# xmed-lab/NEURONS

Measured on AMD Instinct MI355X. Metric: denoising frames/sec, 16f x 256^2 clip, 50 DDIM steps, higher is better.
Workload: dtype bf16; 1 GPU; BASELINE config 2: 1 clip(s) per call, (1,4,16,32,32) latent, 50 DDIM steps, CFG 8.5 (batch 2), SparseCtrl + temporal U-Net per step, random-init weights; clips_per_gpu=5, ddim_steps=50, hip_graph=True, output_finite=True, attention=bf16

## Files before the change

### neurons_amd/csrc/gemm.hip

```cpp
#include "launchers.h"
#include "device_prims.h"
#include <cstdio>
#include <cstdlib>
#include <utility>

namespace {

__device__ __forceinline__ void glds16_builtin(const void* src, void* lds_wave_base) {
  __builtin_amdgcn_global_load_lds((gptr_t)src, (lptr_t)lds_wave_base, 16, 0, 0);
}

NR_STAMP_BUF(nr_stamp_buf, 512, 48);
#define NR_STAMP_AT(slot) NR_STAMP_PUT(nr_stamp_buf, slot)
#define NR_STAMP_RT(slot) NR_STAMP_PUT_RT(nr_stamp_buf, slot)

template <int BM, int BN, int NS, int WGM, int WGN, bool LNF = false, bool ADMA = false, bool LIN = LNF, bool PH = false>
__global__ __launch_bounds__(64 * WGM * WGN, (LNF && WGM * WGN == 8) ? 4 : 1) void igemm_bf16_kernel(NrGemmParams p_arg, int splitk, float* partial, int m_fast) {
  NrGemmParams p = nr_pin_params(p_arg);
  if constexpr (LIN) { p.ksize = 1; p.stride = 1; p.ups = 0; p.a1 = nullptr; p.c1 = 0; p.tap_inner = 0; p.pad_tl0 = 0; }
  static_assert(!PH || (!LIN && !LNF), "the phase form is a conv");
  if constexpr (PH) { p.ksize = 3; p.stride = 1; p.ups = 2; p.a1 = nullptr; p.c1 = 0; p.tap_inner = 0; p.pad_tl0 = 0; p.geglu = 0; p.rowvec = nullptr; p.res = nullptr; }
  splitk = nr_pin(splitk); partial = nr_pin(partial); m_fast = nr_pin(m_fast);
  constexpr int BK = 64;
  constexpr int NW = WGM * WGN;
  constexpr int WM = BM / WGM, WN = BN / WGN;
  constexpr int MT = WM / 16, NT = WN / 16;
  constexpr int GA = BM / (8 * NW), GB = BN / (8 * NW);
  static_assert(BM % (8 * NW) == 0 && BN % (8 * NW) == 0, "tile rows must split evenly over the waves");
  constexpr int TILE = (BM + BN) * BK;
  extern __shared__ __attribute__((aligned(16))) bf16 smem[];

  const int tid = threadIdx.x;
  const int lane = tid & 63;
  const int wave = tid >> 6;
  NR_STAMP_AT(0);
  NR_STAMP_RT(44);
  const int wm = wave / WGN, wn = wave % WGN;
  const int ntn = (p.N + BN - 1) / BN;
  const int Mrows = PH ? p.M >> 2 : p.M;
  const int ntmp = (Mrows + BM - 1) / BM;
  const int ntm = PH ? 4 * ntmp : ntmp;
  int bid = nr_xcd_bid();
  const int slice = splitk > 1 ? nr_fdiv_small(bid, ntn * ntm) : 0;
  bid -= slice * ntn * ntm;
  int bm, bn;
  if (m_fast >= 2) {
    const int G = m_fast;
    const int band = nr_fdiv_small(bid, G * ntn);
    const int first = band * G;
    const int gsz = min(G, ntm - first);
    const int r = bid - band * G * ntn;
    bn = nr_fdiv_small(r, gsz);
    bm = first + r - bn * gsz;
  } else if (m_fast) { bn = nr_fdiv_small(bid, ntm); bm = bid - bn * ntm; } else { bm = nr_fdiv_small(bid, ntn); bn = bid - bm * ntn; }
  const int phase = PH ? nr_fdiv_small(bm, ntmp) : 0;
  if constexpr (PH) bm -= phase * ntmp;
  const int ph_py = phase >> 1, ph_px = phase & 1;
  const int m0 = bm * BM, n0 = bn * BN;
  auto ph_out_row = [&](int r) {
    const int hw = p.H * p.W;
    const int n = nr_fdiv_small(r, hw);
    const int q = r - n * hw;
    const int y = nr_fdiv_small(q, p.W), x = q - y * p.W;
    return (n * p.OH + 2 * y + ph_py) * p.OW + 2 * x + ph_px;
  };
  NR_STAMP_AT(40);
  const int lr = lane >> 3;
  const int lp = lane & 7;
  const int lchunk = (lp ^ lr) << 3;

  const int Cin = p.c0 + p.c1;

  int a_pix[GA], a_oy[GA], a_ox[GA];
  bool a_ok[GA];
#pragma unroll
  for (int j = 0; j < GA; ++j) {
    const int m = m0 + 8 * (wave * GA + j) + lr;
    a_ok[j] = m < Mrows;
    const int mm = a_ok[j] ? m : 0;
    if constexpr (PH) {
      const int hw = p.H * p.W;
      const int n = nr_fdiv_small(mm, hw);
      const int r = mm - n * hw;
      a_pix[j] = n; a_oy[j] = nr_fdiv_small(r, p.W); a_ox[j] = r - a_oy[j] * p.W;
    } else if (p.ksize == 1) {
      a_pix[j] = mm; a_oy[j] = 0; a_ox[j] = 0;
    } else {
      const int ohw = p.OH * p.OW;
      const int n = nr_fdiv_small(mm, ohw);
      const int r = mm - n * ohw;
      a_pix[j] = n; a_oy[j] = nr_fdiv_small(r, p.OW); a_ox[j] = r - a_oy[j] * p.OW;
    }
  }
  const bf16* zsrc = (const bf16*)nr_zero16;
  const bool tap_inner = !LNF && p.tap_inner != 0;
  long long a_cbyte[GA];
  unsigned a_tapmask[GA];
  if (tap_inner) {
#pragma unroll
    for (int j = 0; j < GA; ++j) {
      a_cbyte[j] = (((long long)a_pix[j] * p.H + a_oy[j]) * p.W + a_ox[j]) * p.lda0 * (long long)sizeof(bf16);
      unsigned msk = 0;
#pragma unroll
      for (int t = 0; t < 9; ++t) {
        const int iy = a_oy[j] + t / 3 - 1, ix = a_ox[j] + t % 3 - 1;
        if (a_ok[j] && iy >= 0 && iy < p.H && ix >= 0 && ix < p.W) msk |= 1u << t;
      }
      a_tapmask[j] = msk;
    }
  }

  NR_STAMP_AT(41);
  const int nk_total = p.K / BK;
  int kt_begin = 0, kt_end = nk_total;
  if (splitk > 1) { kt_begin = nr_fdiv_small(nk_total * slice, splitk); kt_end = nr_fdiv_small(nk_total * (slice + 1), splitk); }

  const bf16* ap[GA];
  int ainc[GA];
  const bf16* wp[GB];
  int winc[GB];
  int st_tap, st_c;
  {
    const int kbase = kt_begin * BK;
    if (tap_inner) { const int q9 = nr_fdiv_small(kt_begin, 9); st_tap = kt_begin - 9 * q9; st_c = q9 * BK; }
    else { st_tap = p.ksize == 3 ? nr_fdiv_small(kbase, Cin) : 0; st_c = kbase - st_tap * Cin; }
#pragma unroll
    for (int j = 0; j < GB; ++j) {
      const int n = n0 + 8 * (wave * GB + j) + lr;
      const bool ok = n < p.N;
      wp[j] = ok ? p.w + ((size_t)phase * p.N + n) * p.K + kbase + lchunk : zsrc;
      winc[j] = ok ? BK : 0;
    }
  }
  auto setup_rows_tap_inner = [&]() {
    const int ky = st_tap / 3, kx = st_tap - ky * 3;
    const long long delta = ((long long)(ky - 1) * p.W + (kx - 1)) * p.lda0 * (long long)sizeof(bf16);
    const char* base = reinterpret_cast<const char*>(p.a0 + st_c + lchunk) + delta;
#pragma unroll
    for (int j = 0; j < GA; ++j) {
      const bool ok = (a_tapmask[j] >> st_tap) & 1u;
      ap[j] = ok ? reinterpret_cast<const bf16*>(base + a_cbyte[j]) : zsrc;
    }
  };
  auto setup_rows = [&]() {
    if (tap_inner) { setup_rows_tap_inner(); return; }
    const bf16* src; int ld;
    if (st_c < p.c0) { src = p.a0 + st_c; ld = p.lda0; } else { src = p.a1 + (st_c - p.c0); ld = p.lda1; }
    src += lchunk;
    if constexpr (PH) {
      const int dy = (st_tap >> 1) + ph_py - 1, dx = (st_tap & 1) + ph_px - 1;
#pragma unroll
      for (int j = 0; j < GA; ++j) {
        const int iy = a_oy[j] + dy, ix = a_ox[j] + dx;
        const bool ok = a_ok[j] && iy >= 0 && iy < p.H && ix >= 0 && ix < p.W;
        const size_t pix = ((size_t)a_pix[j] * p.H + iy) * p.W + ix;
        ap[j] = ok ? src + pix * ld : zsrc;
        ainc[j] = ok ? BK : 0;
      }
    } else if (p.ksize == 1) {
#pragma unroll
      for (int j = 0; j < GA; ++j) {
        ap[j] = a_ok[j] ? src + (size_t)a_pix[j] * ld : zsrc;
        ainc[j] = a_ok[j] ? BK : 0;
      }
    } else {
      const int ky = st_tap / 3, kx = st_tap - ky * 3;
      const int VH = p.ups ? p.H * 2 : p.H, VW = p.ups ? p.W * 2 : p.W;
#pragma unroll
      for (int j = 0; j < GA; ++j) {
        int iy = a_oy[j] * p.stride + ky - (p.pad_tl0 ? 0 : 1);
        int ix = a_ox[j] * p.stride + kx - (p.pad_tl0 ? 0 : 1);
        const bool ok = a_ok[j] && iy >= 0 && iy < VH && ix >= 0 && ix < VW;
        if (p.ups) { iy >>= 1; ix >>= 1; }
        const size_t pix = ((size_t)a_pix[j] * p.H + iy) * p.W + ix;
        ap[j] = ok ? src + pix * ld : zsrc;
        ainc[j] = ok ? BK : 0;
      }
    }
  };
  NR_STAMP_AT(42);
  setup_rows();
  NR_STAMP_AT(43);

  auto stage = [&](int buf) {
    bf16* sA = smem + buf * TILE;
    bf16* sB = sA + BM * BK;
    if constexpr (ADMA) {
      const unsigned la = nr_lds_addr(sA + wave * GA * 8 * BK), lb = nr_lds_addr(sB + wave * GB * 8 * BK);
#pragma unroll
      for (int j = 0; j < GA; ++j) nr_glds16(ap[j], la + (unsigned)(j * 8 * BK * (int)sizeof(bf16)));
#pragma unroll
      for (int j = 0; j < GB; ++j) nr_glds16(wp[j], lb + (unsigned)(j * 8 * BK * (int)sizeof(bf16)));
    } else {
#pragma unroll
      for (int j = 0; j < GA; ++j) glds16_builtin(ap[j], sA + (wave * GA + j) * 8 * BK);
#pragma unroll
      for (int j = 0; j < GB; ++j) glds16_builtin(wp[j], sB + (wave * GB + j) * 8 * BK);
    }
#pragma unroll
    for (int j = 0; j < GB; ++j) wp[j] += winc[j];
    if (tap_inner) {
      st_tap += 1;
      if (st_tap == 9) { st_tap = 0; st_c += BK; }
      setup_rows_tap_inner();
      return;
    }
    st_c += BK;
    bool resetup = false;
    if (st_c == Cin) { st_c = 0; st_tap += 1; resetup = true; }
    else if (p.c1 > 0 && st_c == p.c0) resetup = true;
    if (resetup) {
      if (st_tap < (PH ? 4 : p.ksize * p.ksize)) setup_rows();
    } else {
#pragma unroll
      for (int j = 0; j < GA; ++j) ap[j] += ainc[j];
    }
  };

  f32x4 acc[NT][MT];
#pragma unroll
  for (int i = 0; i < NT; ++i)
#pragma unroll
    for (int j = 0; j < MT; ++j) acc[i][j] = f32x4{0.f, 0.f, 0.f, 0.f};

  const int fr = lane & 15, fg = lane >> 4;
  float ln_s1[MT], ln_s2[MT];
#pragma unroll
  for (int j = 0; j < MT; ++j) { ln_s1[j] = 0.f; ln_s2[j] = 0.f; }
  float* ln_stat = reinterpret_cast<float*>(smem + NS * TILE);

  constexpr int G = GA + GB;
#pragma unroll
  for (int s0 = 0; s0 < NS - 1; ++s0)
    if (kt_begin + s0 < kt_end) stage(s0);
  int cur = 0;
  NR_STAMP_AT(1);
  for (int kt = kt_begin; kt < kt_end; ++kt) {
    if (kt + (NS - 2) < kt_end) nr_wait_vmcnt<(NS - 2) * G>(); else nr_wait_vmcnt<0>();
    __builtin_amdgcn_s_barrier();
    NR_STAMP_AT(4 + (kt - kt_begin));
    const bf16* sA = smem + cur * TILE;
    const bf16* sB = sA + BM * BK;
    bf16x8 wf[2][NT], xf[2][MT];
#pragma unroll
    for (int i = 0; i < NT; ++i) {
      const int row = wn * WN + i * 16 + fr;
      wf[0][i] = *(const bf16x8*)(sB + row * BK + ((fg ^ (row & 7)) << 3));
    }
#pragma unroll
    for (int j = 0; j < MT; ++j) {
      const int row = wm * WM + j * 16 + fr;
      xf[0][j] = *(const bf16x8*)(sA + row * BK + ((fg ^ (row & 7)) << 3));
    }
    __builtin_amdgcn_sched_barrier(0);
    {
      const int nxt = kt + NS - 1;
      int nb = cur + NS - 1; if (nb >= NS) nb -= NS;
      if (nxt < kt_end) stage(nb);
    }
    __builtin_amdgcn_sched_barrier(0);
#pragma unroll
    for (int i = 0; i < NT; ++i) {
      const int row = wn * WN + i * 16 + fr;
      wf[1][i] = *(const bf16x8*)(sB + row * BK + (((4 + fg) ^ (row & 7)) << 3));
    }
#pragma unroll
    for (int j = 0; j < MT; ++j) {
      const int row = wm * WM + j * 16 + fr;
      xf[1][j] = *(const bf16x8*)(sA + row * BK + (((4 + fg) ^ (row & 7)) << 3));
    }
#pragma unroll
    for (int ks = 0; ks < 2; ++ks)
#pragma unroll
      for (int i = 0; i < NT; ++i)
#pragma unroll
        for (int j = 0; j < MT; ++j)
          acc[i][j] = __builtin_amdgcn_mfma_f32_16x16x32_bf16(wf[ks][i], xf[ks][j], acc[i][j], 0, 0, 0);
    if constexpr (LNF) {
      const bf16x2 one2 = {(bf16)1.0f, (bf16)1.0f};
#pragma unroll
      for (int ks = 0; ks < 2; ++ks) {
        if (((2 * kt + ks) & (WGN - 1)) != wn) continue;
#pragma unroll
        for (int j = 0; j < MT; ++j)
#pragma unroll
          for (int e = 0; e < 4; ++e) {
            const bf16x2 pr = {xf[ks][j][2 * e], xf[ks][j][2 * e + 1]};
            ln_s2[j] = __builtin_amdgcn_fdot2_f32_bf16(pr, pr, ln_s2[j], false);
            ln_s1[j] = __builtin_amdgcn_fdot2_f32_bf16(pr, one2, ln_s1[j], false);
          }
      }
    }
    cur = cur + 1 == NS ? 0 : cur + 1;
  }
  NR_STAMP_AT(2);
  float ln_mu[MT], ln_rs[MT];
  if constexpr (LNF) {
#pragma unroll
    for (int j = 0; j < MT; ++j) {
      float a = ln_s1[j], b = ln_s2[j];
      a += __shfl_xor(a, 16, 64); b += __shfl_xor(b, 16, 64);
      a += __shfl_xor(a, 32, 64); b += __shfl_xor(b, 32, 64);
      if (fg == 0) {
        const int row = wm * WM + j * 16 + fr;
        ln_stat[(0 * WGN + wn) * BM + row] = a;
        ln_stat[(1 * WGN + wn) * BM + row] = b;
      }
    }
    __syncthreads();
#pragma unroll
    for (int j = 0; j < MT; ++j) {
      const int row = wm * WM + j * 16 + fr;
      float a = 0.f, b = 0.f;
#pragma unroll
      for (int w = 0; w < WGN; ++w) { a += ln_stat[(0 * WGN + w) * BM + row]; b += ln_stat[(1 * WGN + w) * BM + row]; }
      const float inv = 1.0f / (float)p.K;
      const float mu = a * inv;
      ln_mu[j] = mu;
      ln_rs[j] = rsqrtf(fmaxf(b * inv - mu * mu, 0.f) + p.ln_eps);
    }
#pragma unroll
    for (int i = 0; i < NT; ++i) {
      const int n = n0 + wn * WN + i * 16 + 4 * fg;
      const f32x4 cn = n < p.N ? *(const f32x4*)(p.ln_c + n) : f32x4{0.f, 0.f, 0.f, 0.f};
#pragma unroll
      for (int j = 0; j < MT; ++j)
#pragma unroll
        for (int r = 0; r < 4; ++r) acc[i][j][r] = ln_rs[j] * (acc[i][j][r] - ln_mu[j] * cn[r]);
    }
  }

  if (partial) {
    float* slab = partial + (size_t)slice * p.M * p.N;
#pragma unroll
    for (int j = 0; j < MT; ++j) {
      const int m = m0 + wm * WM + j * 16 + fr;
      if (m >= Mrows) continue;
      const int ms = PH ? phase * Mrows + m : m;
#pragma unroll
      for (int i = 0; i < NT; ++i) {
        const int n = n0 + wn * WN + i * 16 + 4 * fg;
        if (n >= p.N) continue;
        nr_store16f(slab + (size_t)ms * p.N + n, acc[i][j]);
      }
    }
    return;
  }
  constexpr bool STAGED = (size_t)BM * BN * sizeof(float) <= (size_t)NS * TILE * sizeof(bf16);
  if constexpr (STAGED) {
    constexpr int NTH = 64 * NW;
    float* sC = reinterpret_cast<float*>(smem);
    __syncthreads();
    const int bno = p.geglu ? BN / 2 : BN;
#pragma unroll
    for (int j = 0; j < MT; ++j) {
      const int row = wm * WM + j * 16 + fr;
      if (!p.geglu) {
#pragma unroll
        for (int i = 0; i < NT; ++i) {
          const int c4 = ((wn * WN + i * 16) >> 2) + fg;
          *(f32x4*)(sC + row * BN + ((c4 ^ (row & 7)) << 2)) = acc[i][j];
        }
      } else {
        if constexpr (NT % 2 == 0) {
#pragma unroll
          for (int i = 0; i < NT; i += 2) {
            const int nv = n0 + wn * WN + i * 16 + 4 * fg;
            f32x4 v = acc[i][j], g = acc[i + 1][j];
            if (p.bias && nv < p.N) { v += *(const f32x4*)(p.bias + nv); g += *(const f32x4*)(p.bias + nv + 16); }
            f32x4 o;
#pragma unroll
            for (int e = 0; e < 4; ++e) o[e] = v[e] * gelu_erf_fast(g[e]);
            const int c4 = (((wn * WN + i * 16) >> 1) >> 2) + fg;
            *(f32x4*)(sC + row * BN + ((c4 ^ (row & 7)) << 2)) = o;
          }
        }
      }
    }
    __syncthreads();
    const int c8n = bno >> 3;
    const int nout = p.geglu ? p.N / 2 : p.N;
    const int nb0 = p.geglu ? n0 / 2 : n0;
    for (int idx = tid; idx < BM * c8n; idx += NTH) {
      const int row = idx / c8n, c8 = idx - row * c8n;
      const int m = m0 + row, n = nb0 + c8 * 8;
      if (m >= Mrows || n >= nout) continue;
      f32x4 va = *(const f32x4*)(sC + row * BN + (((2 * c8) ^ (row & 7)) << 2));
      f32x4 vb = *(const f32x4*)(sC + row * BN + (((2 * c8 + 1) ^ (row & 7)) << 2));
      if (!p.geglu) {
        if (p.bias) { va += *(const f32x4*)(p.bias + n); vb += *(const f32x4*)(p.bias + n + 4); }
        if (p.rowvec) {
          const float* rv = p.rowvec + nr_rowvec_row(p, m) + n;
          va += *(const f32x4*)rv; vb += *(const f32x4*)(rv + 4);
        }
        va *= p.out_scale; vb *= p.out_scale;
        if (p.act == 1) {
#pragma unroll
          for (int e = 0; e < 4; ++e) { va[e] = quick_gelu_f(va[e]); vb[e] = quick_gelu_f(vb[e]); }
        }
        if (p.res) {
          const bf16x8 r = *(const bf16x8*)(p.res + (size_t)m * p.ldr + n);
#pragma unroll
          for (int e = 0; e < 4; ++e) { va[e] += (float)r[e]; vb[e] += (float)r[4 + e]; }
        }
      }
      bf16x8 o;
#pragma unroll
      for (int e = 0; e < 4; ++e) { o[e] = (bf16)va[e]; o[4 + e] = (bf16)vb[e]; }
      nr_store16(p.out + (size_t)(PH ? ph_out_row(m) : m) * p.ldo + n, o);
    }
#ifdef NR_STAMP
    asm volatile("s_waitcnt vmcnt(0)" ::: "memory");
#endif
    NR_STAMP_AT(3);
    NR_STAMP_RT(45);
    return;
  }
#pragma unroll
  for (int j = 0; j < MT; ++j) {
    const int m = m0 + wm * WM + j * 16 + fr;
    if (m >= Mrows) continue;
    const size_t mo = PH ? ph_out_row(m) : m;
    const float* rv = p.rowvec ? p.rowvec + nr_rowvec_row(p, m) : nullptr;
    if (!p.geglu) {
#pragma unroll
      for (int i = 0; i < NT; ++i) {
        const int n = n0 + wn * WN + i * 16 + 4 * fg;
        if (n >= p.N) continue;
        f32x4 v = acc[i][j];
        if (p.bias) { const f32x4 b = *(const f32x4*)(p.bias + n); v += b; }
        if (rv) { const f32x4 t = *(const f32x4*)(rv + n); v += t; }
        v *= p.out_scale;
        if (p.act == 1) {
#pragma unroll
          for (int e = 0; e < 4; ++e) v[e] = quick_gelu_f(v[e]);
        }
        if (p.res) {
          const bf16x4 r = *(const bf16x4*)(p.res + (size_t)m * p.ldr + n);
#pragma unroll
          for (int e = 0; e < 4; ++e) v[e] += (float)r[e];
        }
        bf16x4 o;
#pragma unroll
        for (int e = 0; e < 4; ++e) o[e] = (bf16)v[e];
        nr_store8(p.out + mo * p.ldo + n, o);
      }
    } else {
      if constexpr (NT % 2 == 0) {
#pragma unroll
        for (int i = 0; i < NT; i += 2) {
          const int nv = n0 + wn * WN + i * 16 + 4 * fg;
          if (nv >= p.N) continue;
          const int ng = nv + 16;
          f32x4 v = acc[i][j], g = acc[i + 1][j];
          if (p.bias) {
            v += *(const f32x4*)(p.bias + nv);
            g += *(const f32x4*)(p.bias + ng);
          }
          const int oc = ((n0 + wn * WN + i * 16) >> 1) + 4 * fg;
          bf16x4 o;
#pragma unroll
          for (int e = 0; e < 4; ++e) o[e] = (bf16)(v[e] * gelu_erf_fast(g[e]));
          nr_store8(p.out + mo * p.ldo + oc, o);
        }
      }
    }
  }
}

template <bool PH>
__global__ __launch_bounds__(256) void splitk_reduce_kernel(NrGemmParams p_arg, int splitk, const float* __restrict__ partial) {
  const NrGemmParams p = nr_pin_params(p_arg);
  const long long idx = (long long)blockIdx.x * 256 + threadIdx.x;
  const int n4 = p.N >> 2;
  if (idx >= (long long)p.M * n4) return;
  const int m = (int)(idx / n4);
  const int n = (int)(idx - (long long)m * n4) << 2;
  const size_t slab = (size_t)p.M * p.N;
  const float* src = partial + (size_t)m * p.N + n;
  f32x4 v = *(const f32x4*)src;
  for (int s = 1; s < splitk; ++s) v += *(const f32x4*)(src + s * slab);
  if (p.bias) v += *(const f32x4*)(p.bias + n);
  if (p.rowvec) v += *(const f32x4*)(p.rowvec + nr_rowvec_row(p, m) + n);
  v *= p.out_scale;
  if (p.act == 1) {
#pragma unroll
    for (int e = 0; e < 4; ++e) v[e] = quick_gelu_f(v[e]);
  }
  if (p.res) {
    const bf16x4 r = *(const bf16x4*)(p.res + (size_t)m * p.ldr + n);
#pragma unroll
    for (int e = 0; e < 4; ++e) v[e] += (float)r[e];
  }
  bf16x4 o;
#pragma unroll
  for (int e = 0; e < 4; ++e) o[e] = (bf16)v[e];
  size_t mo = (size_t)m;
  if constexpr (PH) {
    const int Mp = p.M >> 2, hw = p.H * p.W;
    const int phase = m / Mp, r = m - phase * Mp;
    const int img = r / hw, q = r - img * hw;
    const int y = q / p.W, x = q - y * p.W;
    mo = (size_t)(img * p.OH + 2 * y + (phase >> 1)) * p.OW + 2 * x + (phase & 1);
  }
  nr_store8(p.out + mo * p.ldo + n, o);
}

typedef TiledPlan Plan;

constexpr unsigned rings(std::initializer_list<int> ns) { unsigned m = 0; for (int n : ns) m |= 1u << n; return m; }
constexpr bool has_ring(unsigned set, int ns) { return ns >= 0 && ns < 32 && (set >> ns & 1); }
struct TileRow {
  int bm, bn, wgm, wgn;
  unsigned ns, ns_ln;
  bool phase;
  constexpr int waves() const { return wgn == 1 ? 41 : wgm * wgn; }
  constexpr size_t lds_bytes(int NS, bool ln) const { return (size_t)NS * (bm + bn) * 64 * sizeof(bf16) + (ln ? (size_t)2 * wgn * bm * sizeof(float) : 0); }
};
constexpr int RING_MIN = 2, RING_MAX = 8, LIN_MAX_RING = 4, PHASE_RING = 2;
constexpr TileRow TILES[] = {
    {256, 160, 2, 2, rings({2, 3}), 0, false},
    {256, 128, 2, 2, rings({2, 3}), 0, false},
    {256, 128, 4, 2, rings({2, 3}), 0, true},
    {128, 160, 4, 1, rings({3, 4}), rings({3, 4}), false},
    {128, 160, 2, 2, rings({2, 3, 4}), 0, true},
    {128, 128, 2, 4, rings({2, 3, 4}), rings({2}), true},
    {128, 128, 2, 2, rings({2, 3, 4}), rings({2}), false},
    {128, 64, 4, 2, rings({2, 3, 4}), rings({2, 4}), false},
    {128, 64, 2, 2, rings({2, 3, 4}), rings({2, 4}), true},
    {64, 160, 2, 2, rings({2, 3, 4}), rings({2, 3}), false},
    {64, 64, 2, 2, rings({2, 3, 4, 6, 8}), rings({2, 4}), true},
    {64, 32, 2, 2, rings({2, 3, 4, 6, 8}), rings({2, 4}), false},
};
constexpr int NTILES = sizeof(TILES) / sizeof(TILES[0]), NRINGS = RING_MAX - RING_MIN + 1;
constexpr bool table_fits_lds() {
  for (const TileRow& t : TILES)
    for (int ns = 0; ns < 32; ++ns)
      if ((has_ring(t.ns, ns) && (ns < RING_MIN || ns > RING_MAX || t.lds_bytes(ns, false) > 160 * 1024)) ||
          (has_ring(t.ns_ln, ns) && (!has_ring(t.ns, ns) || t.lds_bytes(ns, true) > 160 * 1024)) || (t.phase && !has_ring(t.ns, PHASE_RING))) return false;
  return true;
}
static_assert(table_fits_lds(), "every ring is RING_MIN .. RING_MAX deep and fits the 160 KiB of a CU's LDS; a LayerNorm-folded depth and the phase depth are depths of the tile");
constexpr const TileRow* find_row(int bm, int bn, int waves, bool phase = false) {
  for (const TileRow& t : TILES)
    if (t.bm == bm && t.bn == bn && (waves == 0 || t.waves() == waves) && (!phase || t.phase)) return &t;
  return nullptr;
}

inline long long row_tiles(const NrGemmParams& p, int bm) { return p.ups == 2 ? 4ll * ((p.M / 4 + bm - 1) / bm) : (p.M + bm - 1) / bm; }

Plan choose_plan_phase(const NrGemmParams& p) {
  auto nblk = [&](int bm, int bn) { return row_tiles(p, bm) * ((p.N + bn - 1) / bn); };
  const int nk = p.K / 64;
  Plan pl{};
  pl.splitk = 1; pl.stages = 2; pl.waves = 4;
  if (p.N % 160 == 0) {
    pl.bm = 128; pl.bn = 160;
    if (p.M <= 2048 && nk >= 64) { pl.splitk = 4; return pl; }
  } else {
    const bool n128 = p.N % 128 == 0 || p.N >= 960;
    if (n128 && nblk(128, 128) >= 400) { pl.bm = 128; pl.bn = 128; pl.waves = 8; }
    else if (nblk(128, 64) >= 256) { pl.bm = 128; pl.bn = 64; }
    else { pl.bm = 64; pl.bn = 64; }
  }
  const long long tiles = nblk(pl.bm, pl.bn);
  if (tiles < 512 && nk >= 64) {
    int s_ = (int)((1024 + tiles - 1) / tiles);
    if (s_ > nk / 16) s_ = nk / 16;
    if (s_ > 4) s_ = 4;
    pl.splitk = s_ < 1 ? 1 : s_;
  }
  return pl;
}
Plan choose_plan(const NrGemmParams& p) {
  auto nblk = [&](int bm, int bn) { return (long long)((p.M + bm - 1) / bm) * ((p.N + bn - 1) / bn); };
  const int nk = p.K / 64;
  Plan pl{};
  pl.splitk = 1; pl.stages = 2; pl.waves = 4;
  if (p.ups == 2) return choose_plan_phase(p);
  if (!p.geglu && p.M <= 1024 && nk >= 128 && p.N % 160 == 0) {
    pl.bm = 128; pl.bn = 160; pl.splitk = nk >= 300 ? 16 : 8;
    return pl;
  }
  if (!p.geglu && p.ksize == 3 && p.M <= 2048 && nk >= 128 && p.N % 160 == 0) {
    pl.bm = 128; pl.bn = 160; pl.splitk = 4;
    return pl;
  }
  if (!p.geglu && p.ksize == 3 && p.M <= 8192 && p.N % 160 == 0 && p.N < 960 && nk >= 64 && nblk(128, 160) >= 128 && nblk(128, 160) < 512) {
    pl.bm = 128; pl.bn = 160; pl.splitk = 2;
    return pl;
  }
  if (!p.geglu && p.ksize == 1 && p.M <= 2048 && p.M > 512 && nk >= 96 && p.N % 160 == 0) {
    pl.bm = 128; pl.bn = 160; pl.splitk = 4;
    return pl;
  }
  static const bool t64x160_rule = env_not_0("NR_IGEMM_T64X160");
  if (t64x160_rule && p.ksize == 1 && !p.geglu && p.N % 160 == 0 && p.M > 512 && nk >= 16 && nk <= 48 && nblk(64, 160) >= 128 && nblk(64, 160) <= 256) {
    pl.bm = 64; pl.bn = 160; pl.stages = 3;
    return pl;
  }
  const bool n128 = p.N % 128 == 0 || p.N >= 960;
  if (!p.geglu && p.N % 160 == 0 && p.N < 960 && p.N % 128 != 0 && nk >= 20 && nblk(128, 160) >= 256) { pl.bm = 128; pl.bn = 160; }
  else if (n128 && nblk(128, 128) >= 400) { pl.bm = 128; pl.bn = 128; pl.waves = 8; }
  else if (nblk(128, 64) >= 512 || (nblk(128, 64) >= 256 && nk > 32)) { pl.bm = 128; pl.bn = 64; pl.waves = nk <= 32 ? 8 : 4; }
  else if (nblk(64, 64) >= 256 && nk <= 96) { pl.bm = 64; pl.bn = 64; }
  else if (p.M >= 1024 && nblk(128, 64) >= 64) { pl.bm = 128; pl.bn = 64; }
  else { pl.bm = 64; pl.bn = 64; }
  static const bool smallm_rule = env_not_0("NR_IGEMM_SMALLM");
  static const bool wide_rule = env_not_0("NR_IGEMM_WIDE");
  static const bool rowwave_rule = env_not_0("NR_IGEMM_ROWWAVE");
  if (smallm_rule && p.ksize == 1 && p.M <= 512 && nk >= 8) {
    pl.bm = 64; pl.bn = p.geglu ? 64 : 32; pl.waves = 4; pl.stages = 4;
    if (p.geglu && p.N >= 8192 && p.M >= 256) { pl.bm = 128; pl.bn = 128; pl.waves = 8; pl.stages = 2; }
    if (rowwave_rule && p.geglu && p.N >= 8192 && p.N % 160 == 0 && p.M > 256 && nblk(128, 160) <= 256) {
      pl.bm = 128; pl.bn = 160; pl.waves = 41; pl.stages = p.ln_c ? 3 : 4;
    }
    else if (!p.geglu && nk >= 96 && !p.ln_c) { pl.bm = 64; pl.bn = 64; pl.stages = 2; pl.splitk = 4; return pl; }
    else if (wide_rule && !p.geglu && nblk(64, 32) > 640 && nblk(128, 64) >= 192) { pl.bm = 128; pl.bn = 64; pl.waves = 8; pl.stages = 4; }
  }
  if (!p.geglu) {
    const long long tiles = nblk(pl.bm, pl.bn);
    const int cap_m = p.M >= 8192 ? 2 : (p.M >= 2048 ? 4 : 8);
    const int min_tiles = p.M <= 1024 ? 8 : 16;
    if (tiles < 512 && nk >= 4 * min_tiles) {
      int s_ = (int)((1280 + tiles - 1) / tiles);
      if (s_ > nk / min_tiles) s_ = nk / min_tiles;
      if (s_ > cap_m) s_ = cap_m;
      if (s_ < 1) s_ = 1;
      pl.splitk = s_;
    }
  }
  return pl;
}

inline NrGemmParams plan_view(const NrGemmParams& p) {
  NrGemmParams q = p;
  q.M = nr_plan_rows(p);
  return q;
}

typedef void (*igemm_kern_t)(NrGemmParams, int, float*, int);

template <int I, int NS>
int launch_inst(const NrGemmParams& p, unsigned grid, const Plan& pl, float* partial, int m_fast, hipStream_t stream) {
  constexpr TileRow T = TILES[I];
  constexpr int BM = T.bm, BN = T.bn, WGM = T.wgm, WGN = T.wgn;
  const bool ln = p.ln_c != nullptr, plain = !ln && p.ups != 2;
  igemm_kern_t k = nullptr;
  int ki = 0;
  if constexpr (has_ring(T.ns_ln, NS))
    if (ln) k = igemm_bf16_kernel<BM, BN, NS, WGM, WGN, true>;
  if constexpr (T.phase && NS == PHASE_RING)
    if (p.ups == 2 && !ln) { k = !pl.adma ? igemm_bf16_kernel<BM, BN, NS, WGM, WGN, false, false, false, true> : igemm_bf16_kernel<BM, BN, NS, WGM, WGN, false, true, false, true>; ki = 5 + pl.adma; }
  if constexpr (has_ring(T.ns, NS))
    if (plain && !pl.lin) { k = !pl.adma ? igemm_bf16_kernel<BM, BN, NS, WGM, WGN, false, false> : igemm_bf16_kernel<BM, BN, NS, WGM, WGN, false, true>; ki = 1 + pl.adma; }
  if constexpr (has_ring(T.ns, NS) && NS <= LIN_MAX_RING)
    if (plain && pl.lin) { k = !pl.adma ? igemm_bf16_kernel<BM, BN, NS, WGM, WGN, false, false, true> : igemm_bf16_kernel<BM, BN, NS, WGM, WGN, false, true, true>; ki = 3 + pl.adma; }
  if (!k) return 9;
  const size_t shm = T.lds_bytes(NS, ln);
  static unsigned long long attr_done[7] = {};
  if (const int rc = nr_lds_opt_in(attr_done[ki], {(const void*)k}, shm)) return rc;
  hipLaunchKernelGGL(k, dim3(grid), dim3(64 * WGM * WGN), shm, stream, p, pl.splitk, partial, m_fast);
  return 0;
}
template <size_t... J>
int launch_exact(std::index_sequence<J...>, const NrGemmParams& p, unsigned grid, const Plan& pl, float* partial, int m_fast, hipStream_t stream) {
  int rc = 9;
  const auto is = [&](const TileRow& t, int ns) { return pl.bm == t.bm && pl.bn == t.bn && pl.waves == t.waves() && pl.stages == ns; };
  (void)((is(TILES[J / NRINGS], RING_MIN + (int)(J % NRINGS)) &&
          ((rc = launch_inst<(int)(J / NRINGS), RING_MIN + (int)(J % NRINGS)>(p, grid, pl, partial, m_fast, stream)), true)) || ...);
  return rc;
}

constexpr int pick_ring(unsigned set, int want) {
  int deepest = 0;
  for (int ns = RING_MIN; ns <= RING_MAX; ++ns)
    if (has_ring(set, ns)) { if (ns >= want) return ns; deepest = ns; }
  return deepest;
}
int legalise(const NrGemmParams& p, Plan& pl) {
  const bool ln = p.ln_c != nullptr, phase = p.ups == 2;
  const bool row_wave = pl.waves == 41;
  if (ln && pl.bn == 32) pl.bn = 64;
  if (!find_row(pl.bm, pl.bn, 0)) return 9;
  const TileRow* t = phase ? find_row(pl.bm, pl.bn, 0, true) : find_row(pl.bm, pl.bn, pl.waves);
  if (!t && !phase) t = find_row(pl.bm, pl.bn, 4);
  if (!t || (ln && !t->ns_ln)) t = find_row(128, 128, 8);
  pl.bm = t->bm; pl.bn = t->bn; pl.waves = t->waves();
  if (phase) pl.stages = PHASE_RING;
  else if (ln) pl.stages = row_wave || has_ring(t->ns_ln, pl.stages) ? pick_ring(t->ns_ln, pl.stages) : 2;
  else pl.stages = pick_ring(t->ns, pl.stages);
  return 0;
}

void apply_override(const NrGemmParams& p, Plan& pl, int& m_fast) {
  const char* e = getenv("NR_IGEMM_FORCE");
  if (!e) return;
  if (const char* f = getenv("NR_IGEMM_FORCE_MAXM")) if (p.M > atoi(f)) return;
  if (const char* f = getenv("NR_IGEMM_FORCE_MINM")) if (p.M < atoi(f)) return;
  if (const char* f = getenv("NR_IGEMM_FORCE_KS")) if (p.ksize != atoi(f)) return;
  if (const char* f = getenv("NR_IGEMM_FORCE_N")) if (p.N != atoi(f)) return;
  if (const char* f = getenv("NR_IGEMM_FORCE_K")) if (p.K != atoi(f)) return;
  int bm = -1, bn = -1, sk = -1, st = -1, ord = -1, wv = -1;
  sscanf(e, "%d,%d,%d,%d,%d,%d", &bm, &bn, &sk, &st, &ord, &wv);
  if (bm > 0 && bn > 0) {
    if (find_row(bm, bn, 0) && !(p.geglu && ((bn == 160 && !(bm == 128 && wv == 41)) || bn == 32))) { pl.bm = bm; pl.bn = bn; }
  }
  if (wv == 4 || wv == 8) pl.waves = wv;
  if (pl.bm == 256 && pl.bn == 128 && wv != 4) pl.waves = 8;
  if (pl.bn == 160 || pl.bm == 64) pl.waves = 4;
  if (wv == 41 && pl.bm == 128 && pl.bn == 160) pl.waves = 41;
  if (sk > 0 && !p.geglu) { const int nk = p.K / 64; pl.splitk = sk > nk ? nk : sk; }
  if (st >= 2 && st <= 8) pl.stages = st;
  if (ord >= 0) m_fast = ord;
}

int tile_order(double w_elems, double a_elems, int ntm, int ntn) {
  static const bool grouped = env_not_0("NR_IGEMM_GROUPED");
  static const double grouped_minw = getenv("NR_IGEMM_GROUPED_MINW") ? atof(getenv("NR_IGEMM_GROUPED_MINW")) : 3.0e6;
  if (grouped && ntm >= 8 && ntn >= 4 && w_elems >= grouped_minw) return 8;
  return w_elems > a_elems ? 1 : 0;
}

int route(const NrGemmParams& p, NrGemmRoute* r, bool packed_ok) {
  std::memset(r, 0, sizeof(*r));
  r->weight_layout = p.tap_inner ? NR_W_TAP_INNER : NR_W_ROWMAJOR;
  const int Cin = p.c0 + p.c1;
  const bool phase = p.ups == 2;
  if (phase) {
    r->cls = NR_GEMM_TILED;
    if (p.ksize != 3 || p.stride != 1 || p.a1 || p.c1 || p.tap_inner || p.pad_tl0 || p.geglu || p.ln_c || p.out_f32 || p.res || p.rowvec) return 10;
    if (p.H < 1 || p.W < 1 || p.OH != 2 * p.H || p.OW != 2 * p.W || p.M < 4 || p.M % (p.OH * p.OW) != 0) return 11;
  } else if (p.ups != 0 && p.ups != 1) return 11;
  if (!phase && packed_ok && smallm_plan(p, &r->smallm)) { r->cls = NR_GEMM_SMALLM; r->weight_layout = p.w8 ? NR_W_FRAGMAJOR_E4M3 : NR_W_FRAGMAJOR; return 0; }
  if (!phase && packed_ok && lin160_plan(p, &r->lin160)) { r->cls = NR_GEMM_LIN160; r->weight_layout = r->lin160.form == 4 ? NR_W_LIN128Q : NR_W_LIN160; return 0; }
  if (!phase && p.K == p.ksize * p.ksize * Cin && rowpanel_plan(p, &r->rowpanel)) { r->cls = NR_GEMM_ROWPANEL; return 0; }
  const double w_elems = (double)p.N * p.K;
  if (!phase && g8p_plan(p, &r->g8p)) {
    r->cls = NR_GEMM_G8P;
    r->m_fast = tile_order(w_elems, (double)p.M * Cin, (p.M + 255) / 256, (p.N + 64 * r->g8p.nt - 1) / (64 * r->g8p.nt));
    return 0;
  }
  r->cls = NR_GEMM_TILED;
  if (p.K % 64 != 0 || Cin % 64 != 0 || p.N % 32 != 0) return 1;
  if (p.a1 && (p.c0 % 64 != 0)) return 2;
  if (p.K != (phase ? 4 : p.ksize * p.ksize) * Cin) return 3;
  if (p.ksize != 1 && p.ksize != 3) return 4;
  if (p.tap_inner && (p.ksize != 3 || p.stride != 1 || p.ups || p.pad_tl0 || p.a1)) return 5;
  Plan& pl = r->tiled;
  pl = choose_plan(plan_view(p));
  const double a_elems = (double)p.M * Cin * (p.ksize == 3 ? (p.stride == 2 ? 4.0 : (p.ups ? 0.25 : 1.0)) : 1.0);
  const int ntm1 = (int)(phase ? row_tiles(p, pl.bm) / 4 : row_tiles(p, pl.bm));
  r->m_fast = tile_order(w_elems, a_elems, ntm1, (p.N + pl.bn - 1) / pl.bn);
  apply_override(p, pl, r->m_fast);
  if (p.ln_c) {
    if (p.ksize != 1 || p.a1 || p.out_f32) return 8;
    pl.splitk = 1;
  }
  if (legalise(p, pl)) return 9;
  if (phase && r->m_fast >= 2 && (row_tiles(p, pl.bm) / 4) % r->m_fast != 0) r->m_fast = w_elems > a_elems ? 1 : 0;
  if (p.out_f32) {
    if (p.geglu) return 7;
    pl.splitk = 1;
  }
  static const int adma_min = getenv("NR_IGEMM_ADMA_MINK") ? atoi(getenv("NR_IGEMM_ADMA_MINK")) : 24;
  static const bool lin_on = env_not_0("NR_IGEMM_LIN");
  pl.adma = (p.K / 64) / (pl.splitk > 1 ? pl.splitk : 1) >= adma_min;
  pl.lin = lin_on && p.ksize == 1 && !p.a1 && p.c1 == 0;
  if (pl.stages > LIN_MAX_RING) pl.lin = 0;
  if (p.ln_c) { pl.adma = 0; pl.lin = 1; }
  r->ws_bytes = pl.splitk > 1 ? (size_t)pl.splitk * p.M * p.N * sizeof(float) : 0;
  return 0;
}

int launch_tiled(const NrGemmParams& p, const Plan& pl, int m_fast, float* workspace, hipStream_t stream) {
  if (pl.splitk < 1 || pl.splitk > p.K / 64 || ((p.ln_c || p.out_f32) && pl.splitk != 1)) return 9;
  if (pl.splitk > 1 && !workspace) return 6;
  float* partial = p.out_f32 ? p.out_f32 : (pl.splitk > 1 ? workspace : nullptr);
  const unsigned grid = (unsigned)(row_tiles(p, pl.bm) * ((p.N + pl.bn - 1) / pl.bn) * pl.splitk);
  if (const int rc = launch_exact(std::make_index_sequence<NTILES * NRINGS>{}, p, grid, pl, partial, m_fast, stream)) return rc;
  if (pl.splitk > 1) {
    const long long total = (long long)p.M * (p.N / 4);
    hipLaunchKernelGGL(p.ups == 2 ? splitk_reduce_kernel<true> : splitk_reduce_kernel<false>, dim3((unsigned)((total + 255) / 256)), dim3(256), 0, stream, p,
                       pl.splitk, (const float*)partial);
  }
  return 0;
}

}

extern "C" int nr_gemm_route(const NrGemmParams* pp, NrGemmRoute* r) { return route(*pp, r, true); }
extern "C" int nr_gemm_route_rowmajor(const NrGemmParams* pp, NrGemmRoute* r) { return route(*pp, r, false); }

extern "C" int nr_launch_gemm(const NrGemmParams* pp, const NrGemmRoute* r, const bf16* packed_w, float* ws, hipStream_t stream) {
  switch (r->cls) {
    case NR_GEMM_SMALLM: return nr_launch_smallm(pp, &r->smallm, packed_w, r->weight_layout, stream);
    case NR_GEMM_LIN160: return nr_launch_lin160(pp, &r->lin160, packed_w, stream);
    case NR_GEMM_ROWPANEL: return nr_launch_rowpanel(pp, &r->rowpanel, stream);
    case NR_GEMM_G8P: return nr_launch_g8p(pp, &r->g8p, r->m_fast, stream);
    case NR_GEMM_TILED: return launch_tiled(*pp, r->tiled, r->m_fast, ws, stream);
  }
  return 9;
}

extern "C" size_t nr_gemm_packed_bytes(int layout, int N, int K) {
  switch (layout) {
    case NR_W_FRAGMAJOR: return (N % 16 == 0 && K % 32 == 0) ? (size_t)N * K * sizeof(bf16) : 0;
    case NR_W_FRAGMAJOR_E4M3: return (N > 0 && K > 0 && N % 16 == 0 && K % 64 == 0) ? (size_t)N * K + (size_t)N * sizeof(float) : 0;
    case NR_W_LIN160: return nr_lin160_stream_bytes(N, K);
    case NR_W_LIN128Q: return nr_lin128q_stream_bytes(N, K);
  }
  return 0;
}
extern "C" int nr_launch_gemm_w_pack(int layout, const bf16* w, int N, int K, bf16* dst, hipStream_t stream) {
  switch (layout) {
    case NR_W_FRAGMAJOR: return nr_launch_smallm_w_pack(w, dst, N, K, stream);
    case NR_W_FRAGMAJOR_E4M3: return nr_launch_smallm_w8_pack(w, dst, N, K, stream);
    case NR_W_LIN160: return nr_launch_lin160_w_pack(w, N, K, dst, stream);
    case NR_W_LIN128Q: return nr_launch_lin128q_w_pack(w, N, K, dst, stream);
  }
  return 1;
}

#ifdef NR_STAMP
extern "C" int nr_stamp_read(void* dst, size_t bytes, int clear) { return nr_stamp_read_buf(nr_stamp_buf, dst, bytes, clear); }
#endif
```

Measured before the change: 20.39 frames/s.

## Add k-pair igemm kernel splitting each tile's K range across two in-block groups

Adds a 512-thread igemm kernel with a 128x160 tile in which two 256-thread groups each accumulate half of a K slice. Each group has its own double-buffered LDS ring, and the two halves are summed through LDS before the epilogue. The planner swaps even split-k 128x160 plans for this form at half the split count. It also routes one specific 1x1 shape (N=640, K=3200) to it. The aim is to halve the fp32 partial slabs and reduce-kernel traffic while keeping CU occupancy. The cost is more LDS per block and a one-block-per-CU launch bound.

```diff
diff --git a/neurons_amd/csrc/gemm.hip b/neurons_amd/csrc/gemm.hip
--- a/neurons_amd/csrc/gemm.hip
+++ b/neurons_amd/csrc/gemm.hip
@@ -468,6 +468,302 @@
   }
 }
 
+template <bool LIN, bool TAPI>
+__global__ __launch_bounds__(512, 1) void igemm_kpair_kernel(NrGemmParams p_arg, int nslab, float* partial, int m_fast) {
+  NrGemmParams p = nr_pin_params(p_arg);
+  static_assert(!(LIN && TAPI), "the tap-inner order is a conv's");
+  p.ups = 0;
+  if constexpr (LIN) { p.ksize = 1; p.stride = 1; p.a1 = nullptr; p.c1 = 0; p.pad_tl0 = 0; }
+  if constexpr (TAPI) { p.ksize = 3; p.stride = 1; p.a1 = nullptr; p.c1 = 0; p.pad_tl0 = 0; }
+  nslab = nr_pin(nslab); partial = nr_pin(partial); m_fast = nr_pin(m_fast);
+  constexpr int BM = 128, BN = 160, BK = 64, WGN = 2, NW = 4;
+  constexpr int WM = 64, WN = 80, MT = WM / 16, NT = WN / 16;
+  constexpr int GA = BM / (8 * NW), GB = BN / (8 * NW);
+  constexpr int TILE = (BM + BN) * BK;
+  extern __shared__ __attribute__((aligned(16))) bf16 smem[];
+
+  const int tid = threadIdx.x;
+  const int lane = tid & 63;
+  const int grp = __builtin_amdgcn_readfirstlane(tid >> 8);
+  const int wave = __builtin_amdgcn_readfirstlane((tid >> 6) & 3);
+  NR_STAMP_AT(0);
+  NR_STAMP_RT(44);
+  const int wm = wave / WGN, wn = wave % WGN;
+  const int ntn = (p.N + BN - 1) / BN;
+  const int ntm = (p.M + BM - 1) / BM;
+  int bid = nr_xcd_bid();
+  const int pair = nslab > 1 ? nr_fdiv_small(bid, ntn * ntm) : 0;
+  bid -= pair * ntn * ntm;
+  int bm, bn;
+  if (m_fast >= 2) {
+    const int G = m_fast;
+    const int band = nr_fdiv_small(bid, G * ntn);
+    const int first = band * G;
+    const int gsz = min(G, ntm - first);
+    const int r = bid - band * G * ntn;
+    bn = nr_fdiv_small(r, gsz);
+    bm = first + r - bn * gsz;
+  } else if (m_fast) { bn = nr_fdiv_small(bid, ntm); bm = bid - bn * ntm; } else { bm = nr_fdiv_small(bid, ntn); bn = bid - bm * ntn; }
+  const int m0 = bm * BM, n0 = bn * BN;
+  const int lr = lane >> 3;
+  const int lp = lane & 7;
+  const int lchunk = (lp ^ lr) << 3;
+  const int Cin = p.c0 + p.c1;
+
+  int a_pix[GA], a_oy[GA], a_ox[GA];
+  bool a_ok[GA];
+#pragma unroll
+  for (int j = 0; j < GA; ++j) {
+    const int m = m0 + 8 * (wave * GA + j) + lr;
+    a_ok[j] = m < p.M;
+    const int mm = a_ok[j] ? m : 0;
+    if (p.ksize == 1) {
+      a_pix[j] = mm; a_oy[j] = 0; a_ox[j] = 0;
+    } else {
+      const int ohw = p.OH * p.OW;
+      const int n = nr_fdiv_small(mm, ohw);
+      const int r = mm - n * ohw;
+      a_pix[j] = n; a_oy[j] = nr_fdiv_small(r, p.OW); a_ox[j] = r - a_oy[j] * p.OW;
+    }
+  }
+  const bf16* zsrc = (const bf16*)nr_zero16;
+  constexpr bool tap_inner = TAPI;
+  long long a_cbyte[GA];
+  unsigned a_tapmask[GA];
+  if constexpr (tap_inner) {
+#pragma unroll
+    for (int j = 0; j < GA; ++j) {
+      a_cbyte[j] = (((long long)a_pix[j] * p.H + a_oy[j]) * p.W + a_ox[j]) * p.lda0 * (long long)sizeof(bf16);
+      unsigned msk = 0;
+#pragma unroll
+      for (int t = 0; t < 9; ++t) {
+        const int iy = a_oy[j] + t / 3 - 1, ix = a_ox[j] + t % 3 - 1;
+        if (a_ok[j] && iy >= 0 && iy < p.H && ix >= 0 && ix < p.W) msk |= 1u << t;
+      }
+      a_tapmask[j] = msk;
+    }
+  }
+
+  const int nk_total = p.K / BK;
+  const int S = 2 * nslab, slice = 2 * pair + grp;
+  const int kt_begin = nr_fdiv_small(nk_total * slice, S), kt_end = nr_fdiv_small(nk_total * (slice + 1), S);
+  const int nmine = kt_end - kt_begin;
+  const int nsib = nr_fdiv_small(nk_total * ((slice ^ 1) + 1), S) - nr_fdiv_small(nk_total * (slice ^ 1), S);
+  const int nmax = max(nmine, nsib);
+
+  const bf16* ap[GA];
+  const bf16* wp[GB];
+  int st_tap, st_c;
+  {
+    const int kbase = kt_begin * BK;
+    if constexpr (tap_inner) { const int q9 = nr_fdiv_small(kt_begin, 9); st_tap = kt_begin - 9 * q9; st_c = q9 * BK; }
+    else { st_tap = p.ksize == 3 ? nr_fdiv_small(kbase, Cin) : 0; st_c = kbase - st_tap * Cin; }
+#pragma unroll
+    for (int j = 0; j < GB; ++j) {
+      const int n = min(n0 + 8 * (wave * GB + j) + lr, p.N - 1);
+      wp[j] = p.w + (size_t)n * p.K + kbase + lchunk;
+    }
+  }
+  auto setup_rows_tap_inner = [&]() {
+    const int ky = st_tap / 3, kx = st_tap - ky * 3;
+    const long long delta = ((long long)(ky - 1) * p.W + (kx - 1)) * p.lda0 * (long long)sizeof(bf16);
+    const char* base = reinterpret_cast<const char*>(p.a0 + st_c + lchunk) + delta;
+#pragma unroll
+    for (int j = 0; j < GA; ++j) {
+      const bool ok = (a_tapmask[j] >> st_tap) & 1u;
+      ap[j] = ok ? reinterpret_cast<const bf16*>(base + a_cbyte[j]) : zsrc;
+    }
+  };
+  auto setup_rows = [&]() {
+    if constexpr (tap_inner) { setup_rows_tap_inner(); return; }
+    const bf16* src; int ld;
+    if (st_c < p.c0) { src = p.a0 + st_c; ld = p.lda0; } else { src = p.a1 + (st_c - p.c0); ld = p.lda1; }
+    src += lchunk;
+    if (p.ksize == 1) {
+#pragma unroll
+      for (int j = 0; j < GA; ++j) {
+        ap[j] = a_ok[j] ? src + (size_t)a_pix[j] * ld : zsrc;
+      }
+    } else {
+      const int ky = st_tap / 3, kx = st_tap - ky * 3;
+#pragma unroll
+      for (int j = 0; j < GA; ++j) {
+        const int iy = a_oy[j] * p.stride + ky - (p.pad_tl0 ? 0 : 1);
+        const int ix = a_ox[j] * p.stride + kx - (p.pad_tl0 ? 0 : 1);
+        const bool ok = a_ok[j] && iy >= 0 && iy < p.H && ix >= 0 && ix < p.W;
+        const size_t pix = ((size_t)a_pix[j] * p.H + iy) * p.W + ix;
+        ap[j] = ok ? src + pix * ld : zsrc;
+      }
+    }
+  };
+  setup_rows();
+
+  bf16* ring = smem + grp * 2 * TILE;
+  auto stage = [&](int buf) {
+    bf16* sA = ring + buf * TILE;
+    bf16* sB = sA + BM * BK;
+    const unsigned la = nr_lds_addr(sA + wave * GA * 8 * BK), lb = nr_lds_addr(sB + wave * GB * 8 * BK);
+#pragma unroll
+    for (int j = 0; j < GA; ++j) nr_glds16(ap[j], la + (unsigned)(j * 8 * BK * (int)sizeof(bf16)));
+#pragma unroll
+    for (int j = 0; j < GB; ++j) nr_glds16(wp[j], lb + (unsigned)(j * 8 * BK * (int)sizeof(bf16)));
+#pragma unroll
+    for (int j = 0; j < GB; ++j) wp[j] += BK;
+    if constexpr (tap_inner) {
+      st_tap += 1;
+      if (st_tap == 9) { st_tap = 0; st_c += BK; }
+      setup_rows_tap_inner();
+      return;
+    }
+    st_c += BK;
+    bool resetup = false;
+    if (st_c == Cin) { st_c = 0; st_tap += 1; resetup = true; }
+    else if (p.c1 > 0 && st_c == p.c0) resetup = true;
+    if (resetup) {
+      if (st_tap < p.ksize * p.ksize) setup_rows();
+    } else {
+#pragma unroll
+      for (int j = 0; j < GA; ++j) ap[j] += ap[j] != zsrc ? BK : 0;
+    }
+  };
+
+  f32x4 acc[NT][MT];
+#pragma unroll
+  for (int i = 0; i < NT; ++i)
+#pragma unroll
+    for (int j = 0; j < MT; ++j) acc[i][j] = f32x4{0.f, 0.f, 0.f, 0.f};
+
+  const int fr = lane & 15, fg = lane >> 4;
+  bf16x8 wf[2][NT], xf[2][MT];
+  auto read_frags = [&](int buf, int ks) {
+    const bf16* sA = ring + buf * TILE;
+    const bf16* sB = sA + BM * BK;
+#pragma unroll
+    for (int i = 0; i < NT; ++i) {
+      const int row = wn * WN + i * 16 + fr;
+      wf[ks][i] = *(const bf16x8*)(sB + row * BK + (((4 * ks + fg) ^ (row & 7)) << 3));
+    }
+#pragma unroll
+    for (int j = 0; j < MT; ++j) {
+      const int row = wm * WM + j * 16 + fr;
+      xf[ks][j] = *(const bf16x8*)(sA + row * BK + (((4 * ks + fg) ^ (row & 7)) << 3));
+    }
+  };
+  auto multiply = [&]() {
+#pragma unroll
+    for (int ks = 0; ks < 2; ++ks)
+#pragma unroll
+      for (int i = 0; i < NT; ++i)
+#pragma unroll
+        for (int j = 0; j < MT; ++j)
+          acc[i][j] = __builtin_amdgcn_mfma_f32_16x16x32_bf16(wf[ks][i], xf[ks][j], acc[i][j], 0, 0, 0);
+  };
+  auto barrier = [&]() {
+    __builtin_amdgcn_sched_barrier(0);
+    __builtin_amdgcn_s_barrier();
+    __builtin_amdgcn_sched_barrier(0);
+  };
+
+  auto load_tile = [&](int t) {
+    if (t < nmine) {
+      read_frags(t & 1, 0);
+      __builtin_amdgcn_sched_barrier(0);
+      if (t + 1 < nmine) stage((t & 1) ^ 1);
+      __builtin_amdgcn_sched_barrier(0);
+      read_frags(t & 1, 1);
+    }
+  };
+  if (nmine > 0) stage(0);
+  NR_STAMP_AT(1);
+  if (grp == 0) {
+    for (int t = 0; t < nmax; ++t) {
+      if (t < nmine) nr_wait_vmcnt<0>();
+      barrier();
+      if (t < 18) NR_STAMP_AT(4 + 2 * t);
+      load_tile(t);
+      barrier();
+      if (t < 18) NR_STAMP_AT(5 + 2 * t);
+      if (t < nmine) multiply();
+    }
+  } else {
+    for (int t = 0; t < nmax; ++t) {
+      barrier();
+      if (t > 0 && t - 1 < nmine) multiply();
+      if (t < nmine) nr_wait_vmcnt<0>();
+      barrier();
+      load_tile(t);
+    }
+    if (nmax - 1 < nmine) multiply();
+  }
+  NR_STAMP_AT(2);
+
+  f32x4* xch = reinterpret_cast<f32x4*>(smem);
+  const int t256 = tid & 255;
+  barrier();
+  if (grp == 1) {
+#pragma unroll
+    for (int i = 0; i < NT; ++i)
+#pragma unroll
+      for (int j = 0; j < MT; ++j) xch[(i * MT + j) * 256 + t256] = acc[i][j];
+    asm volatile("s_waitcnt lgkmcnt(0)" ::: "memory");
+  }
+  barrier();
+  if (grp == 1) return;
+#pragma unroll
+  for (int i = 0; i < NT; ++i)
+#pragma unroll
+    for (int j = 0; j < MT; ++j) acc[i][j] = acc[i][j] + xch[(i * MT + j) * 256 + t256];
+
+  if (partial) {
+    float* slab = partial + (size_t)pair * p.M * p.N;
+#pragma unroll
+    for (int j = 0; j < MT; ++j) {
+      const int m = m0 + wm * WM + j * 16 + fr;
+      if (m >= p.M) continue;
+#pragma unroll
+      for (int i = 0; i < NT; ++i) {
+        const int n = n0 + wn * WN + i * 16 + 4 * fg;
+        if (n >= p.N) continue;
+        nr_store16f(slab + (size_t)m * p.N + n, acc[i][j]);
+      }
+    }
+    return;
+  }
+#pragma unroll
+  for (int j = 0; j < MT; ++j) {
+    const int m = m0 + wm * WM + j * 16 + fr;
+    if (m >= p.M) continue;
+    const float* rv = p.rowvec ? p.rowvec + nr_rowvec_row(p, m) : nullptr;
+#pragma unroll
+    for (int i = 0; i < NT; ++i) {
+      const int n = n0 + wn * WN + i * 16 + 4 * fg;
+      if (n >= p.N) continue;
+      f32x4 v = acc[i][j];
+      if (p.bias) { const f32x4 b = *(const f32x4*)(p.bias + n); v += b; }
+      if (rv) { const f32x4 t = *(const f32x4*)(rv + n); v += t; }
+      v *= p.out_scale;
+      if (p.act == 1) {
+#pragma unroll
+        for (int e = 0; e < 4; ++e) v[e] = quick_gelu_f(v[e]);
+      }
+      if (p.res) {
+        const bf16x4 r = *(const bf16x4*)(p.res + (size_t)m * p.ldr + n);
+#pragma unroll
+        for (int e = 0; e < 4; ++e) v[e] += (float)r[e];
+      }
+      bf16x4 o;
+#pragma unroll
+      for (int e = 0; e < 4; ++e) o[e] = (bf16)v[e];
+      nr_store8(p.out + (size_t)m * p.ldo + n, o);
+    }
+  }
+#ifdef NR_STAMP
+  asm volatile("s_waitcnt vmcnt(0)" ::: "memory");
+#endif
+  NR_STAMP_AT(3);
+  NR_STAMP_RT(45);
+}
+
 template <bool PH>
 __global__ __launch_bounds__(256) void splitk_reduce_kernel(NrGemmParams p_arg, int splitk, const float* __restrict__ partial) {
   const NrGemmParams p = nr_pin_params(p_arg);
@@ -572,7 +868,7 @@
   }
   return pl;
 }
-Plan choose_plan(const NrGemmParams& p) {
+Plan choose_plan_slices(const NrGemmParams& p) {
   auto nblk = [&](int bm, int bn) { return (long long)((p.M + bm - 1) / bm) * ((p.N + bn - 1) / bn); };
   const int nk = p.K / 64;
   Plan pl{};
@@ -629,6 +925,29 @@
       if (s_ < 1) s_ = 1;
       pl.splitk = s_;
     }
+  }
+  return pl;
+}
+
+constexpr int KPAIR_WAVES = 82;
+inline bool kpair_ok(const NrGemmParams& p, const Plan& pl) {
+  return pl.waves == KPAIR_WAVES && !p.ln_c && !p.geglu && !p.ups && !p.out_f32 && pl.bm == 128 && pl.bn == 160 && pl.splitk >= 1 && 2 * pl.splitk <= p.K / 64;
+}
+inline void kpair_undo(Plan& pl) { if (pl.waves == KPAIR_WAVES) { pl.waves = 4; pl.splitk *= 2; } }
+
+Plan choose_plan(const NrGemmParams& p) {
+  const Plan pl = choose_plan_slices(p);
+  static const bool kpair_rule = env_not_0("NR_IGEMM_KPAIR");
+  if (!kpair_rule) return pl;
+  const long long tiles = (long long)((p.M + 127) / 128) * ((p.N + 159) / 160);
+  Plan kp = pl;
+  kp.waves = KPAIR_WAVES;
+  if (pl.bm == 128 && pl.bn == 160 && pl.waves == 4 && pl.stages == 2 && pl.splitk >= 2 && pl.splitk % 2 == 0) {
+    kp.splitk = pl.splitk / 2;
+    if (tiles * kp.splitk >= 256 && kpair_ok(p, kp)) return kp;
+  } else if (p.ksize == 1 && pl.bm == 128 && pl.bn == 64 && pl.waves == 4 && pl.stages == 2 && pl.splitk == 1 && p.N == 640 && p.K == 3200 && tiles == 256) {
+    kp.bm = 128; kp.bn = 160;
+    if (kpair_ok(p, kp)) return kp;
   }
   return pl;
 }
@@ -672,6 +991,15 @@
   return rc;
 }
 
+int launch_kpair(const NrGemmParams& p, unsigned grid, const Plan& pl, float* partial, int m_fast, hipStream_t stream) {
+  const igemm_kern_t k = pl.lin ? igemm_kpair_kernel<true, false> : (p.tap_inner ? igemm_kpair_kernel<false, true> : igemm_kpair_kernel<false, false>);
+  const size_t shm = (size_t)2 * 2 * (128 + 160) * 64 * sizeof(bf16);
+  static unsigned long long attr_done[3] = {};
+  if (const int rc = nr_lds_opt_in(attr_done[pl.lin ? 0 : (p.tap_inner ? 1 : 2)], {(const void*)k}, shm)) return rc;
+  hipLaunchKernelGGL(k, dim3(grid), dim3(512), shm, stream, p, pl.splitk, partial, m_fast);
+  return 0;
+}
+
 constexpr int pick_ring(unsigned set, int want) {
   int deepest = 0;
   for (int ns = RING_MIN; ns <= RING_MAX; ++ns)
@@ -681,6 +1009,10 @@
 int legalise(const NrGemmParams& p, Plan& pl) {
   const bool ln = p.ln_c != nullptr, phase = p.ups == 2;
   const bool row_wave = pl.waves == 41;
+  if (pl.waves == KPAIR_WAVES) {
+    pl.stages = 2;
+    return kpair_ok(p, pl) ? 0 : 9;
+  }
   if (ln && pl.bn == 32) pl.bn = 64;
   if (!find_row(pl.bm, pl.bn, 0)) return 9;
   const TileRow* t = phase ? find_row(pl.bm, pl.bn, 0, true) : find_row(pl.bm, pl.bn, pl.waves);
@@ -703,6 +1035,7 @@
   if (const char* f = getenv("NR_IGEMM_FORCE_K")) if (p.K != atoi(f)) return;
   int bm = -1, bn = -1, sk = -1, st = -1, ord = -1, wv = -1;
   sscanf(e, "%d,%d,%d,%d,%d,%d", &bm, &bn, &sk, &st, &ord, &wv);
+  kpair_undo(pl);
   if (bm > 0 && bn > 0) {
     if (find_row(bm, bn, 0) && !(p.geglu && ((bn == 160 && !(bm == 128 && wv == 41)) || bn == 32))) { pl.bm = bm; pl.bn = bn; }
   }
@@ -711,6 +1044,13 @@
   if (pl.bn == 160 || pl.bm == 64) pl.waves = 4;
   if (wv == 41 && pl.bm == 128 && pl.bn == 160) pl.waves = 41;
   if (sk > 0 && !p.geglu) { const int nk = p.K / 64; pl.splitk = sk > nk ? nk : sk; }
+  if (wv == KPAIR_WAVES) {
+    Plan kp = pl;
+    kp.waves = KPAIR_WAVES;
+    if (sk <= 0) kp.splitk = pl.splitk >= 2 ? pl.splitk / 2 : 1;
+    if (2 * kp.splitk > p.K / 64) kp.splitk = p.K / 128;
+    if (kpair_ok(p, kp)) pl = kp;
+  }
   if (st >= 2 && st <= 8) pl.stages = st;
   if (ord >= 0) m_fast = ord;
 }
@@ -765,7 +1105,7 @@
   }
   static const int adma_min = getenv("NR_IGEMM_ADMA_MINK") ? atoi(getenv("NR_IGEMM_ADMA_MINK")) : 24;
   static const bool lin_on = env_not_0("NR_IGEMM_LIN");
-  pl.adma = (p.K / 64) / (pl.splitk > 1 ? pl.splitk : 1) >= adma_min;
+  pl.adma = pl.waves == KPAIR_WAVES || (p.K / 64) / (pl.splitk > 1 ? pl.splitk : 1) >= adma_min;
   pl.lin = lin_on && p.ksize == 1 && !p.a1 && p.c1 == 0;
   if (pl.stages > LIN_MAX_RING) pl.lin = 0;
   if (p.ln_c) { pl.adma = 0; pl.lin = 1; }
@@ -775,10 +1115,13 @@
 
 int launch_tiled(const NrGemmParams& p, const Plan& pl, int m_fast, float* workspace, hipStream_t stream) {
   if (pl.splitk < 1 || pl.splitk > p.K / 64 || ((p.ln_c || p.out_f32) && pl.splitk != 1)) return 9;
+  const bool kpair = pl.waves == KPAIR_WAVES;
+  if (kpair && !(kpair_ok(p, pl) && pl.stages == 2)) return 9;
   if (pl.splitk > 1 && !workspace) return 6;
   float* partial = p.out_f32 ? p.out_f32 : (pl.splitk > 1 ? workspace : nullptr);
   const unsigned grid = (unsigned)(row_tiles(p, pl.bm) * ((p.N + pl.bn - 1) / pl.bn) * pl.splitk);
-  if (const int rc = launch_exact(std::make_index_sequence<NTILES * NRINGS>{}, p, grid, pl, partial, m_fast, stream)) return rc;
+  if (const int rc = kpair ? launch_kpair(p, grid, pl, partial, m_fast, stream)
+                           : launch_exact(std::make_index_sequence<NTILES * NRINGS>{}, p, grid, pl, partial, m_fast, stream)) return rc;
   if (pl.splitk > 1) {
     const long long total = (long long)p.M * (p.N / 4);
     hipLaunchKernelGGL(p.ups == 2 ? splitk_reduce_kernel<true> : splitk_reduce_kernel<false>, dim3((unsigned)((total + 255) / 256)), dim3(256), 0, stream, p,
```

New measurement: 20.60 frames/s (median of 6 runs). 1.01x the previous value.
